# aschneuw/road-segmentation-unet

Hardware: AMD Instinct MI355X
Metric: 388x388 patches/sec fwd+bwd (1/2/4/8 GPU) + conv MFMA % of peak (higher is better)
Workload: dtype bf16; 1 GPU; U-Net fwd+bwd+momentum step, num_layers=5 root_size=64 patch_size=388 input=572; batch_per_gpu=4, global_batch=4, parallelism=dp1

## Files before the change

### road_segmentation_unet_amd/csrc/igemm.h

```cpp
#pragma once
#include "rsu_common.h"

struct IgSrc {
    const bf16_t* ptr;
    int H, W, C;
    int oy, ox;
};

struct IgFwdParams {
    IgSrc src[3];
    int nsrc;
    int nchunk[3];
    const bf16_t* wp;
    long wp_y_stride;
    int ntiles_w;
    int tile_off;
    const float* bias;
    bf16_t* out;
    const bf16_t* mask_src;
    bf16_t* pool_out;
    unsigned char* pool_code;
    const void* zero_page;
    int N, Hin, Win;
    int Ho, Wo;
    int Cout;
    int outC;
    int dil, stride, pad;
    int oH, oW, ostride;
    int relu, accumulate;
    int ncob;
    int lsw;
    int ksplit, cob_group;
    float* kslab;
    long kslab_stride;
    int dbg;
    unsigned* stamps;
    TileGeo g;
};

struct IgFwdCfgInfo { int TN, TM, threads; };
enum { IGF2_CFG_128x256 = 0, IGF2_CFG_64x512 = 1, IGF2_CFG_128x128 = 2, IGF2_CFG_64x256 = 3, IGF2_CFG_128x192 = 4, IGF2_CFG_64x384 = 5,
       IGF2_CFG_128x320 = 6, IGF2_CFG_64x640 = 7, IGF2_NCFG = 8 };
IgFwdCfgInfo igemm_fwd2_cfg_info(int cfg);
int igemm_fwd2_max_pieces(int cfg, int ntap);
size_t igemm_fwd2_lds_bytes(int cfg, int ntap, int npix_max);
hipError_t igemm_fwd2_launch(int cfg, int ntap, const IgFwdParams& p, int grid_x, int grid_y, hipStream_t st);
hipError_t igemm_pp_launch(int cfg, const IgFwdParams& p, int grid_x, hipStream_t st);
hipError_t igemm_pp_d2_launch(int cfg, const IgFwdParams& p, int grid_x, hipStream_t st);
bool igemm_pp_d2_supports(int cfg, const IgFwdParams& p);
bool igemm_pp_has(int cfg);
bool igemm_pp_has_ksplit(int cfg);
bool igemm_pp_supports(int cfg, const IgFwdParams& p);
int igemm_pp_pool_lsw_mask(int cfg);
size_t igemm_pp_slab_floats(int cfg, const IgFwdParams& p);
hipError_t igemm_pp_finish_launch(int cfg, const IgFwdParams& p, hipStream_t st);

struct IgCtParams {
    const bf16_t* a;
    int Ca;
    int nchunk;
    int N, H, W;
    unsigned magic_hw, magic_w;
    const bf16_t* wp;
    long wp_phase_stride;
    int ntiles_w;
    const float* bias;
    bf16_t* out;
    int outC;
    int Cn;
    const bf16_t* mask_src;
    int ncob, nnb;
};
bool igemm_ct_supports(int mode, int N, int H, int W, int Ca, int Cn);
hipError_t igemm_ct_launch(int mode, const IgCtParams& p, int grid_x, hipStream_t st);
hipError_t conv_first_fwd_launch(const void* in16, const void* wp, int ntiles_w, const float* bias, void* y, int N, int H, int W, int Cout, int dil,
                                 int relu, int ncu, hipStream_t st, const float* x = nullptr, const float* cw = nullptr, const float* cb = nullptr);

struct IgWgradParams {
    const bf16_t* F;
    int Hf, Wf, Cf;
    IgSrc S;
    float* slab;
    float* bslab;
    float* sbslab;
    long slab_stride;
    int CsOut, CfOut, cs_off;
    const void* zero_page;
    int N, dil, stride;
    int nsplit, ntiles_total;
    int lsw;
    int nbuf, nsw;
    int dbg;
    TileGeo g;
};
enum { IGW_CFG_64x64 = 0, IGW_CFG_64x16 = 1, IGW_CFG_128x64 = 2, IGW_NCFG = 3 };
size_t igemm_wgrad_lds_bytes(int cfg, int npix_max, int nbuf);
int igemm_wgrad_nsw(int cfg, int npix_max);
int igemm_wgrad_tmk(int cfg);
int igemm_wgrad_cfb(int cfg);
int igemm_wgrad_csb(int cfg);
int igemm_wgrad_kgroups(int cfg);
hipError_t igemm_wgrad_launch(int cfg, int ntap, const IgWgradParams& p, int grid_x, int grid_y, int grid_z,
                              hipStream_t st);
bool igemm_wgt_supports(int N, int H, int W, int Cin, int Cout);
int igemm_wgt_blocks(int Cin, int Cout);
int igemm_wgt_tiles(int N, int H, int W);
hipError_t igemm_wgt_launch(const void* x, const void* dy, float* slab, float* sbslab, long slab_stride, int N, int H, int W, int Cin, int Cout,
                            int nsplit, hipStream_t st);
bool igemm_wg1_supports(int N, int H, int W, int Cout, int dil);
int igemm_wg1_blocks(int Cout);
int igemm_wg1_tiles(int N, int Ho, int Wo);
hipError_t igemm_wg1_launch(const void* in16, const void* dz, float* slab, float* bslab, long slab_stride, int N, int H, int W, int Cout, int dil,
                            int nsplit, hipStream_t st);
enum { IGW_FAM_WGPP3 = 0, IGW_FAM_WGPP4 = 1, IGW_FAM_WGPP5 = 2, IGW_FAM_WGPP6 = 3, IGW_FAM_WGP64_4 = 4, IGW_FAM_WGP64_5 = 5,
       IGW_FAM_GENERIC = 8  };
#define IGW_GROUP_MAX 16
#define IGW_UNITS_MAX 2048
struct IgWgJob {
    IgWgradParams p;
    int gx, gy, gz;
    int family;
    int pad_;
};
struct IgWgGroupParams {
    int njobs, nwg;
    IgWgJob job[IGW_GROUP_MAX];
    int wg_first[257];
    unsigned unit[IGW_UNITS_MAX];
};
int igemm_wg_group_family(int cfg, int ntap, const IgWgradParams& p);
size_t igemm_wg_group_lds_bytes(int family, const IgWgradParams& p);
#define IGW_GROUP_LDS_BYTES (160 * 1024)
hipError_t igemm_wg_group_launch(const IgWgGroupParams* dev_table, int nwg_total, hipStream_t st);
bool igemm_wgpp_supports(int cfg, int ntap, const IgWgradParams& p);
bool igemm_wgp64_supports(int cfg, int ntap, const IgWgradParams& p);
hipError_t igemm_wgp64_launch(const IgWgradParams& p, int gx, int gy, int gz, hipStream_t st);
hipError_t igemm_wgpp_launch(const IgWgradParams& p, int grid_x, int grid_y, int grid_z, hipStream_t st);
```

### road_segmentation_unet_amd/csrc/igemm_ct.hip

```cpp
#include <type_traits>

#include "igemm.h"

#define RSU_SENT 0x80000000u

namespace {
__device__ __forceinline__ void bdma16c(__amdgpu_buffer_rsrc_t rsrc, unsigned voff, unsigned soff, void* lds_wave_base) {
    __builtin_amdgcn_raw_ptr_buffer_load_lds(rsrc, (__attribute__((address_space(3))) void*)lds_wave_base, 16, voff, soff, 0, 0);
}
}

template <int MODE>
__global__ void __launch_bounds__(512) __attribute__((amdgpu_waves_per_eu(2, 2))) igemm_ct_kernel(const IgCtParams p) {
    constexpr int NW = 8, CT = 4, PT = 4, TM = 256, TN = 128, WPX = 4;
    constexpr int APL = TM * 64, WPL = (TN / 16) * 1024;
    constexpr int SLOT = 2 * APL + 2 * WPL, NSLOT = 3;
    constexpr int NST = (CT / 2) * PT;
    constexpr int NPW = 6;
    extern __shared__ __attribute__((aligned(16))) char smem[];
    __attribute__((address_space(3))) char* lds = (__attribute__((address_space(3))) char*)smem;
    constexpr int bias_base = NSLOT * SLOT;

    const int lane = threadIdx.x & 63;
    const int wave = __builtin_amdgcn_readfirstlane(threadIdx.x >> 6);
    const int grp = wave >> 2, w4 = wave & 3;
    const int wco = wave / WPX, wpx = wave % WPX;
    const int g4 = lane >> 4, l15 = lane & 15, lq = lane >> 2;
    auto sgpr = [](auto v) { return __builtin_amdgcn_readfirstlane(v); };

    int vid = xcd_contiguous_id(blockIdx.x, gridDim.x);
    const int cob = vid % p.ncob;
    const int tile0 = vid / p.ncob, tstride = gridDim.x / p.ncob;
    const int M = p.N * p.H * p.W;
    const int ntile_m = (M + TM - 1) / TM;
    const int my_tiles = tile0 < ntile_m ? (ntile_m - tile0 + tstride - 1) / tstride : 0;
    if (my_tiles == 0) return;
    const int pha = MODE == 0 ? cob / p.nnb : 0, nb = MODE == 0 ? cob - pha * p.nnb : cob;
    const int ncols = MODE == 0 ? 2 * p.Cn : p.Cn;
    const int NS = MODE == 0 ? (p.nchunk + 1) / 2 : 4 * ((p.nchunk + 1) / 2);
    const int GS = my_tiles * NS;

    int boff[PT];
#pragma unroll
    for (int pt = 0; pt < PT; ++pt) {
        const int hp = (wpx * PT + pt) * 16 + l15;
        boff[pt] = (hp << 6) + ((g4 ^ ((hp >> 1) & 2)) << 4);
    }
    const int afrag = 2 * APL + (wco * CT * 64 + lane) * 16;
    auto mk = [&](const void* ptr) { return __builtin_amdgcn_make_buffer_rsrc((void*)ptr, 0, 0x7fffffff, 0x00020000); };

    const int wG = nb * 4 + w4;
    const bool wvalid = wG * 32 < ncols;
    unsigned w_base;
    if (MODE == 0) {
        const int b = (wG * 32) / p.Cn, lg = (wG * 32 - b * p.Cn) >> 5;
        w_base = sgpr((unsigned)(((long)(pha * 2 + b) * p.wp_phase_stride) * 2 + (long)lg * 2048));
    } else {
        w_base = sgpr((unsigned)(wG * 2048));
    }
    const unsigned w_blk = sgpr((unsigned)(p.ntiles_w * 1024));
    const unsigned w_lane = wvalid ? (unsigned)(lane * 16) : RSU_SENT;
    const int kg8 = ((lane & 3) ^ ((lq >> 1) & 2)) * 8;
    unsigned a_lane[MODE == 0 ? 1 : 4];
    if (MODE == 0) a_lane[0] = (unsigned)((lq * p.Ca + kg8) * 2);
    const int HW = p.H * p.W;
    auto pix_decode = [&](int m, int& n, int& y, int& x) {
        n = (int)__umulhi((unsigned)m, p.magic_hw);
        int r = m - n * HW;
        if (r >= HW) { ++n; r -= HW; }
        y = (int)__umulhi((unsigned)r, p.magic_w);
        x = r - y * p.W;
        if (x >= p.W) { ++y; x -= p.W; }
    };
    int pf_tile = 0;
    int pf_s = 0;
    int pf_slot = 0;
    auto pf_m0 = [&]() { return sgpr((tile0 + pf_tile * tstride) * TM); };
    auto pf_setup_tile = [&]() {
        if (MODE == 1) {
            const int m0 = pf_m0();
#pragma unroll
            for (int q = 0; q < 4; ++q) {
                const int m = m0 + (w4 * 4 + q) * 16 + lq;
                int n, y, x;
                pix_decode(m < M ? m : 0, n, y, x);
                a_lane[q] = m < M ? (unsigned)((((n * 2 * p.H + 2 * y) * 2 * p.W + 2 * x) * p.Ca + kg8) * 2) : RSU_SENT;
            }
        }
    };
    auto pf_issue = [&]() {
        const int st = MODE == 0 ? pf_s : (pf_s >> 2) ;
        const int tap = MODE == 0 ? 0 : (pf_s & 3);
        const int chunk = 2 * st + grp;
        const bool cvalid = chunk < p.nchunk;
        const int crem = p.Ca - chunk * 32;
        const __amdgpu_buffer_rsrc_t ra = mk(p.a), rw = mk(p.wp);
        const int dstA = pf_slot * SLOT + grp * APL, dstW = pf_slot * SLOT + 2 * APL + grp * WPL;
        const int m0 = pf_m0();
        if (MODE == 0) {
            const unsigned soff = sgpr((unsigned)(((long)(m0 + w4 * 64) * p.Ca + chunk * 32) * 2));
            const unsigned pstep = (unsigned)(16 * p.Ca * 2);
            const bool full = cvalid && crem >= 32 && m0 + TM <= M;
#pragma unroll
            for (int q = 0; q < 4; ++q) {
                unsigned vo = a_lane[0];
                if (!full) vo = (cvalid && kg8 < crem && m0 + (w4 * 4 + q) * 16 + lq < M) ? a_lane[0] : RSU_SENT;
                bdma16c(ra, vo, soff + q * pstep, (void*)(lds + dstA + (w4 * 4 + q) * 1024));
            }
        } else {
            const int ta = tap >> 1, tb = tap & 1;
            const unsigned soff = sgpr((unsigned)(((ta * 2 * p.W + tb) * p.Ca + chunk * 32) * 2));
            const bool full = cvalid && crem >= 32;
#pragma unroll
            for (int q = 0; q < 4; ++q) {
                unsigned vo = a_lane[q];
                if (!full) vo = (cvalid && kg8 < crem) ? a_lane[q] : RSU_SENT;
                bdma16c(ra, vo, soff, (void*)(lds + dstA + (w4 * 4 + q) * 1024));
            }
        }
        {
            const unsigned soff = sgpr(w_base + (unsigned)(MODE == 0 ? chunk : chunk * 4 + tap) * w_blk);
            const unsigned vo = cvalid ? w_lane : RSU_SENT;
            bdma16c(rw, vo, soff, (void*)(lds + dstW + (w4 * 2) * 1024));
            bdma16c(rw, vo == RSU_SENT ? RSU_SENT : vo + 1024, soff, (void*)(lds + dstW + (w4 * 2 + 1) * 1024));
        }
        pf_slot = pf_slot == NSLOT - 1 ? 0 : pf_slot + 1;
        if (++pf_s == NS) {
            pf_s = 0;
            if (pf_tile + 1 < my_tiles) ++pf_tile;
            pf_setup_tile();
        }
    };

    if (threadIdx.x < TN) {
        const int col = nb * TN + threadIdx.x;
        float bv = 0.f;
        if (MODE == 0 && p.bias && col < ncols) bv = p.bias[col >= p.Cn ? col - p.Cn : col];
        *(__attribute__((address_space(3))) float*)(lds + bias_base + threadIdx.x * 4) = bv;
    }
    asm volatile("s_waitcnt vmcnt(0)" ::: "memory");
#define CT_STORE(R, VOFF) \
    asm volatile("s_nop 4\n\tbuffer_store_dwordx4 %0, %1, %2, %3 offen\n\ts_nop 3" ::"v"(R), "v"(VOFF), "s"(orsrc), "s"(sbase) : "memory")
    unsigned ovoff[PT];
    const int colw = nb * TN + wco * (CT / 2) * 32;
    auto epi_setup_tile = [&](int m0) {
#pragma unroll
        for (int pt = 0; pt < PT; ++pt) {
            const int m = m0 + (wpx * PT + pt) * 16 + l15;
            if (MODE == 0) {
                int n, y, x;
                pix_decode(m < M ? m : 0, n, y, x);
                ovoff[pt] = m < M ? (unsigned)((((n * 2 * p.H + 2 * y + pha) * 2 * p.W + 2 * x) * p.outC + colw + 8 * g4) * 2) : RSU_SENT;
            } else {
                ovoff[pt] = m < M ? (unsigned)((((wpx * PT + pt) * 16 + l15) * p.outC + colw + 8 * g4) * 2) : RSU_SENT;
            }
        }
    };
    auto epilogue = [&](int m0, f32x4(&acc)[CT][PT]) {
        const __amdgpu_buffer_rsrc_t orsrc = mk(p.out);
        const __amdgpu_buffer_rsrc_t mrsrc = mk(p.mask_src ? (const void*)p.mask_src : (const void*)p.out);
        const unsigned sbase = MODE == 0 ? 0u : sgpr((unsigned)((long)m0 * p.outC * 2));
        unsigned ones_pk = 0x00010001u;
        asm volatile("" : "+v"(ones_pk));
        unsigned voffs[NST];
        u32x4 mk4[NST];
#pragma unroll
        for (int e = 0; e < NST; ++e) {
            const int pt = e / (CT / 2), pp = e % (CT / 2);
            const bool cok = colw + pp * 32 + 8 * g4 < ncols;
            voffs[e] = (cok && ovoff[pt] != RSU_SENT) ? ovoff[pt] + pp * 64 : RSU_SENT;
        }
        if (MODE == 1 && p.mask_src) {
#pragma unroll
            for (int e = 0; e < NST; ++e) mk4[e] = __builtin_amdgcn_raw_buffer_load_b128(mrsrc, voffs[e], sbase, 0);
        }
#pragma unroll
        for (int e = 0; e < NST; ++e) {
            const int pt = e / (CT / 2), pp = e % (CT / 2);
            u32x4 r;
#pragma unroll
            for (int i = 0; i < 2; ++i) {
                r[i] = pack_bf2(acc[2 * pp][pt][2 * i], acc[2 * pp][pt][2 * i + 1]);
                r[2 + i] = pack_bf2(acc[2 * pp + 1][pt][2 * i], acc[2 * pp + 1][pt][2 * i + 1]);
            }
            if (MODE == 1 && p.mask_src) {
#pragma unroll
                for (int i = 0; i < 4; ++i) r[i] &= pos_mask_pk_bf16(mk4[e][i], ones_pk);
            }
            CT_STORE(r, voffs[e]);
        }
    };
    auto bar = [&]() {
        asm volatile("" ::: "memory");
        __builtin_amdgcn_s_barrier();
        asm volatile("" ::: "memory");
    };

    pf_setup_tile();
    pf_issue();
    pf_issue();
    asm volatile("s_waitcnt vmcnt(0) lgkmcnt(0)" ::: "memory");
    bar();
    if (grp) bar();

    f32x4 acc[CT][PT];
    auto run_stream = [&](auto gconst) {
        constexpr int G = decltype(gconst)::value;
        int sit = 0;
        int ck = 0;
        bool after_epi = false;
        epi_setup_tile((tile0 + 0 * tstride) * TM);
        auto phase = [&](auto slotc) {
            constexpr int SL = decltype(slotc)::value;
            if (sit == 0) {
#pragma unroll
                for (int ct = 0; ct < CT; ++ct) {
                    const f32x4 bv = *(const __attribute__((address_space(3))) f32x4*)(lds + bias_base +
                                                                                         ((wco * (CT / 2) + (ct >> 1)) * 32 + 8 * g4 + (ct & 1) * 4) * 4);
#pragma unroll
                    for (int pt = 0; pt < PT; ++pt) {
                        acc[ct][pt] = bv;
                        asm volatile("" : "+v"(acc[ct][pt]));
                    }
                }
            }
            bf16x8 fa[2][CT], fb[2][PT];
#pragma unroll
            for (int ks = 0; ks < 2; ++ks) {
#pragma unroll
                for (int ct = 0; ct < CT; ++ct)
                    fa[ks][ct] = *(const __attribute__((address_space(3))) bf16x8*)(lds + afrag + (SL * SLOT + ks * WPL + ct * 1024));
#pragma unroll
                for (int pt = 0; pt < PT; ++pt)
                    fb[ks][pt] = *(const __attribute__((address_space(3))) bf16x8*)(lds + boff[pt] + (SL * SLOT + ks * APL));
            }
            pf_issue();
            if constexpr (G == 1) {
                if (after_epi) asm volatile("s_waitcnt vmcnt(%0)" ::"n"(NPW + NST) : "memory");
                else asm volatile("s_waitcnt vmcnt(%0)" ::"n"(NPW) : "memory");
            }
            asm volatile("s_waitcnt lgkmcnt(0)" ::: "memory");
            bar();
            __builtin_amdgcn_sched_barrier(0);
            __builtin_amdgcn_s_setprio(1);
#pragma unroll
            for (int ks = 0; ks < 2; ++ks)
#pragma unroll
                for (int pt = 0; pt < PT; ++pt)
#pragma unroll
                    for (int ct = 0; ct < CT; ++ct) mfma_bf16_inplace(acc[ct][pt], fa[ks][ct], fb[ks][pt]);
            __builtin_amdgcn_s_setprio(0);
            __builtin_amdgcn_sched_barrier(0);
            if constexpr (G == 0) {
                if (after_epi) asm volatile("s_waitcnt vmcnt(%0)" ::"n"(NPW + NST) : "memory");
                else asm volatile("s_waitcnt vmcnt(%0)" ::"n"(NPW) : "memory");
            }
            after_epi = false;
            if (sit == NS - 1) mfma_results_fence();
            bar();
            if (sit == NS - 1) {
                const int m0 = sgpr((tile0 + ck * tstride) * TM);
                epilogue(m0, acc);
                after_epi = true;
                sit = 0;
                ++ck;
                if (ck < my_tiles) epi_setup_tile((tile0 + ck * tstride) * TM);
            } else {
                ++sit;
            }
        };
        for (int gs = 0; gs < GS; gs += 3) {
            phase(std::integral_constant<int, 0>{});
            if (gs + 1 >= GS) break;
            phase(std::integral_constant<int, 1>{});
            if (gs + 2 >= GS) break;
            phase(std::integral_constant<int, 2>{});
        }
    };
    if (grp) run_stream(std::integral_constant<int, 1>{}); else run_stream(std::integral_constant<int, 0>{});
    if (!grp) bar();
    asm volatile("s_waitcnt vmcnt(0)" ::: "memory");
}

static size_t ct_lds_bytes() { return 3 * (2 * 256 * 64 + 2 * 8 * 1024) + 512; }

template <int MODE>
static hipError_t ct_launch_one(const IgCtParams& p, int gx, hipStream_t st) {
    auto kern = igemm_ct_kernel<MODE>;
    static bool set = false;
    if (!set) {
        hipError_t e = hipFuncSetAttribute((const void*)kern, hipFuncAttributeMaxDynamicSharedMemorySize, (int)ct_lds_bytes());
        if (e != hipSuccess) return e;
        set = true;
    }
    hipLaunchKernelGGL(kern, dim3(gx), dim3(512), ct_lds_bytes(), st, p);
    return hipGetLastError();
}
bool igemm_ct_supports(int mode, int N, int H, int W, int Ca, int Cn) {
    if (mode == 0 && (Cn % 32)) return false;
    return (long)N * H * W < (1L << 24) && Ca % 8 == 0 && Cn % 8 == 0 && H >= 1 && W >= 1;
}
hipError_t igemm_ct_launch(int mode, const IgCtParams& p, int gx, hipStream_t st) {
    return mode == 0 ? ct_launch_one<0>(p, gx, st) : ct_launch_one<1>(p, gx, st);
}
```

### road_segmentation_unet_amd/csrc/rsu_api.hip

```cpp
#include <array>
#include <atomic>
#include <cmath>
#include <cstdlib>
#include <cstring>
#include <algorithm>
#include <cstddef>
#include <map>
#include <mutex>
#include <vector>

#include "../../include/rsu.h"
#include "../../include/rsu_optim.h"
#include "../../include/rsu_loss.h"
#include "../../include/rsu_cldice.h"
#include "../../include/rsu_lovasz.h"
#include "../../include/rsu_components.h"
#include "../../include/rsu_distance.h"
#include "../../include/rsu_thin.h"
#include "affine_patches.h"
#include "color_jitter.h"
#include "border_map.h"
#include "elementwise.h"
#include "head.h"
#include "cldice.h"
// ... 690 lines not shown
            } ev;
            HIP_CHECK_RET(hipEventCreate(&ev.a));
            HIP_CHECK_RET(hipEventCreate(&ev.b));
            const hipEvent_t e0 = ev.a, e1 = ev.b;
            HIP_CHECK_RET(hipDeviceSynchronize());
            float best_ms = 1e30f, model_ms = 1e30f;
            int best_cfg = pl2.cfg | (pp << 8);
            const int model_code = best_cfg;
            for (int cfg = 0; cfg < IGF2_NCFG; ++cfg) {
                if (igemm_fwd2_cfg_info(cfg).TN != tn_model) continue;
                Fwd2Plan pc;
                if (!plan_fwd2(pc, ncu, N, Ho, Wo, Cout, ntap, kh, kw, dil, stride, gy, ktot, cfg, pool)) continue;
                IgFwdParams pt = p;
                apply_plan(pt, pc);
                for (int vpp = 0; vpp < 2; ++vpp) {
                    if (vpp == 1 && !(pp_ok && !accumulate && pp_supports(cfg, pt))) continue;
                    if (vpp == 0 && pool) continue;
                    if (!vpp && gen >= 4 && pp_ok && !accumulate && pp_supports(cfg, pt)) continue;
                    float ms_min = 1e30f;
                    for (int rep = 0; rep < 6; ++rep) {
                        HIP_CHECK_RET(hipEventRecord(e0, st));
                        HIP_CHECK_RET(launch_persistent(vpp, pc.cfg, ntap, pt, pc.grid_x, gy, st));
                        HIP_CHECK_RET(hipEventRecord(e1, st));
                        HIP_CHECK_RET(hipEventSynchronize(e1));
                        float ms = 0.f;
                        HIP_CHECK_RET(hipEventElapsedTime(&ms, e0, e1));
                        if (rep > 0 && ms < ms_min) ms_min = ms;
                    }
                    if (env_int("RSU_PLAN_DEBUG", 0)) fprintf(stderr, "[tune fwd2] cfg%d pp%d %.1f us\n", cfg, vpp, ms_min * 1e3f);
                    const int code = cfg | (vpp << 8);
                    if (code == model_code) model_ms = ms_min;
                    if (ms_min < best_ms) {
                        best_ms = ms_min;
                        best_cfg = code;
                    }
                }
            }
            if (best_ms > 0.97f * model_ms) best_cfg = model_code;
            if (env_int("RSU_PLAN_DEBUG", 0)) fprintf(stderr, "[tune fwd2] model cfg%d pp%d -> measured cfg%d pp%d\n", pl2.cfg, (int)pp, best_cfg & 255, best_cfg >> 8);
            std::lock_guard<std::mutex> lk(g_tune_mutex);
            g_tuned[tkey] = best_cfg;
            return RSU_OK;
        }
        HIP_CHECK_RET(launch_persistent(pp, pl2.cfg, ntap, p, pl2.grid_x, gy, st));
        return RSU_OK;
    }
}

extern "C" size_t rsu_conv_splitk_ws_floats(void) { return (size_t)256 * 128 * 256 + 1024; }
extern "C" int rsu_conv2d_fwd_k(const rsu_src_t* srcs, int nsrc, const void* packed_fwd, const float* bias, void* y, int N, int Hin,
                                int Win, int Cout, int dil, int relu, int ncu, float* kws, size_t kws_floats, rsu_stream_t stream) {
    if (!srcs || nsrc < 1 || nsrc > 3 || !packed_fwd || !y || Cout % 8 || (dil != 1 && dil != 2)) return RSU_EINVAL;
    const int Ho = Hin - 2 * dil, Wo = Win - 2 * dil;
    if (Ho < 1 || Wo < 2) return RSU_EINVAL;
    return run_fwd(srcs, nsrc, packed_fwd, 0, rup(Cout, 128) / 16, 0, bias, y, nullptr, N, Hin, Win, Ho, Wo, Cout, Cout, 9, 3, dil, 1, 0,
                   Ho, Wo, 1, 1, relu, 0, ncu, (hipStream_t)stream, nullptr, nullptr, kws, kws_floats);
}
extern "C" int rsu_conv2d_fwd(const rsu_src_t* srcs, int nsrc, const void* packed_fwd, const float* bias, void* y, int N, int Hin,
                              int Win, int Cout, int dil, int relu, int ncu, rsu_stream_t stream) {
    return rsu_conv2d_fwd_k(srcs, nsrc, packed_fwd, bias, y, N, Hin, Win, Cout, dil, relu, ncu, nullptr, 0, stream);
}

extern "C" int rsu_conv2d_fwd_pool_k(const rsu_src_t* srcs, int nsrc, const void* packed_fwd, const float* bias, void* y, void* pooled, void* code,
                                     int N, int Hin, int Win, int Cout, float keep, unsigned key, int ncu, float* kws, size_t kws_floats, rsu_stream_t stream);
extern "C" int rsu_conv2d_fwd_pool(const rsu_src_t* srcs, int nsrc, const void* packed_fwd, const float* bias, void* y, void* pooled, void* code,
                                   int N, int Hin, int Win, int Cout, float keep, unsigned key, int ncu, rsu_stream_t stream) {
    return rsu_conv2d_fwd_pool_k(srcs, nsrc, packed_fwd, bias, y, pooled, code, N, Hin, Win, Cout, keep, key, ncu, nullptr, 0, stream);
}
extern "C" int rsu_conv2d_fwd_pool_k(const rsu_src_t* srcs, int nsrc, const void* packed_fwd, const float* bias, void* y, void* pooled, void* code,
                                     int N, int Hin, int Win, int Cout, float keep, unsigned key, int ncu, float* kws, size_t kws_floats, rsu_stream_t stream) {
    if (!srcs || nsrc < 1 || nsrc > 3 || !packed_fwd || !y || !pooled || Cout % 8 || !keep_ok(keep)) return RSU_EINVAL;
    const int Ho = Hin - 2, Wo = Win - 2;
    if (Ho < 2 || Wo < 2) return RSU_EINVAL;
    if (code && ((Ho | Wo) & 1)) return RSU_EINVAL;
    const bool even = ((Ho | Wo) & 1) == 0;
    const int fuse = env_int("RSU_POOL_FUSED", 1);
    bool worth = fuse >= 2;
    if (fuse == 1) {
        Fwd2Plan a, b;
        const int n = launch_ncu(ncu), kt = 0;
        int ktot = 0;
        for (int i = 0; i < nsrc; ++i) ktot += rup(srcs[i].C, 32) * 9;
        (void)kt;
        Fwd2Plan sp;
        worth = n > 0 && !(kws && plan_split(sp, N, Ho, Wo, Cout, ktot, kws_floats)) &&
                plan_fwd2(a, n, N, Ho, Wo, Cout, 9, 3, 3, 1, 1, 1, ktot, -1, false) &&
                plan_fwd2(b, n, N, Ho, Wo, Cout, 9, 3, 3, 1, 1, 1, ktot, -1, true) && b.cost <= 1.08 * a.cost;
    }
    if (keep == 1.f && even && worth && env_int("RSU_FWD_GEN", 3) >= 3 && env_int("RSU_FWD2_CFG", -1) < 0) {
        const int rc = run_fwd(srcs, nsrc, packed_fwd, 0, rup(Cout, 128) / 16, 0, bias, y, nullptr, N, Hin, Win, Ho, Wo, Cout, Cout, 9, 3, 1, 1, 0, Ho, Wo,
                               1, 1, 1, 0, ncu, (hipStream_t)stream, pooled, code);
        if (rc != RSU_EINVAL) return rc;
    }
    const int rc = rsu_conv2d_fwd_k(srcs, nsrc, packed_fwd, bias, y, N, Hin, Win, Cout, 1, 1, ncu, kws, kws_floats, stream);
    if (rc != RSU_OK) return rc;
    return rsu_maxpool2x2_fwd_code(y, pooled, code, N, Ho, Wo, Cout, keep, key, stream);
}

extern "C" size_t rsu_packed_first_bytes(int Cout) {
    int seg[1] = {3};
    return rsu_packed_bytes(9, Cout, seg, 1);
}
extern "C" int rsu_pack_conv_first(const float* w, void* packed, int Cout, rsu_stream_t stream) {
    int seg[1] = {3};
    return do_pack(w, packed, 9, Cout, seg, 1, (long)3 * Cout, 1, Cout, 0, (hipStream_t)stream);
}
extern "C" int rsu_conv_first_fwd(const void* in16, const void* packed, const float* b, void* y, int N, int H, int W, int Cout, int dil,
                                  int ncu, rsu_stream_t stream) {
    if (!in16 || !packed || !y || Cout % 8 || H <= 2 * dil || W <= 2 * dil + 1 || (dil != 1 && dil != 2)) return RSU_EINVAL;
    rsu_src_t s;
    s.ptr = in16; s.H = H; s.W = W; s.C = 16; s.oy = 0; s.ox = 0;
    const int Ho = H - 2 * dil, Wo = W - 2 * dil;
    if (env_int("RSU_FIRST_GEN", 1) != 0) {
        const int n = launch_ncu(ncu);
        if (n < 0) return RSU_EINVAL;
        if ((long)N * Ho * Wo * Cout * 2 >= 0x7ffffff0L || (long)N * H * W * 32 >= 0x7ffffff0L) return RSU_E2BIG;
        HIP_CHECK_RET(conv_first_fwd_launch(in16, packed, rup(Cout, 128) / 16, b, y, N, H, W, Cout, dil, 1, n, (hipStream_t)stream));
        return RSU_OK;
    }
    return run_fwd(&s, 1, packed, 0, rup(Cout, 128) / 16, 0, b, y, nullptr, N, H, W, Ho, Wo, Cout, Cout, 9, 3, dil, 1, 0, Ho, Wo, 1, 1, 1, 0,
                   ncu, (hipStream_t)stream);
}

extern "C" int rsu_color_conv_first_fwd(const float* x, const float* w0, const float* b0, const void* packed, const float* b, void* y, int N, int H,
                                        int W, int Cout, int dil, int ncu, rsu_stream_t stream) {
    if (!x || !w0 || !b0 || !packed || !y || Cout % 8 || H <= 2 * dil || W <= 2 * dil + 1 || (dil != 1 && dil != 2)) return RSU_EINVAL;
    const int Ho = H - 2 * dil, Wo = W - 2 * dil;
    const int n = launch_ncu(ncu);
    if (n < 0) return RSU_EINVAL;
    if ((long)N * Ho * Wo * Cout * 2 >= 0x7ffffff0L || (long)N * H * W * 12 >= 0x7ffffff0L) return RSU_E2BIG;
    HIP_CHECK_RET(conv_first_fwd_launch(nullptr, packed, rup(Cout, 128) / 16, b, y, N, H, W, Cout, dil, 1, n, (hipStream_t)stream, x, w0, b0));
    return RSU_OK;
}

extern "C" int rsu_conv2d_bwd_data_k(const void* dz, const void* packed_bwd, void* dx, const void* relu_src, int accumulate, int N, int H,
                                     int W, int Cin_total, int ci_off, int ci_cnt, int Cout, int dil, int ncu, float* kws, size_t kws_floats, rsu_stream_t stream);
extern "C" int rsu_conv2d_bwd_data(const void* dz, const void* packed_bwd, void* dx, const void* relu_src, int accumulate, int N, int H,
                                   int W, int Cin_total, int ci_off, int ci_cnt, int Cout, int dil, int ncu, rsu_stream_t stream) {
    return rsu_conv2d_bwd_data_k(dz, packed_bwd, dx, relu_src, accumulate, N, H, W, Cin_total, ci_off, ci_cnt, Cout, dil, ncu, nullptr, 0, stream);
}
extern "C" int rsu_conv2d_bwd_data_k(const void* dz, const void* packed_bwd, void* dx, const void* relu_src, int accumulate, int N, int H,
                                     int W, int Cin_total, int ci_off, int ci_cnt, int Cout, int dil, int ncu, float* kws, size_t kws_floats, rsu_stream_t stream) {
    if (!dz || !packed_bwd || !dx || Cout % 8 || ci_cnt % 8 || ci_off % 32 || ci_off + ci_cnt > Cin_total || (dil != 1 && dil != 2))
        return RSU_EINVAL;
    const int Hd = H - 2 * dil, Wd = W - 2 * dil;
    if (Hd < 1 || Wd < 1 || W < 2) return RSU_EINVAL;
    rsu_src_t s;
    s.ptr = dz; s.H = Hd; s.W = Wd; s.C = Cout; s.oy = 0; s.ox = 0;
    return run_fwd(&s, 1, packed_bwd, 0, rup(Cin_total, 128) / 16, ci_off / 16, nullptr, dx, relu_src, N, Hd, Wd, H, W, ci_cnt, ci_cnt, 9,
                   3, dil, 1, 2 * dil, H, W, 1, 1, 0, accumulate, ncu, (hipStream_t)stream, nullptr, nullptr, kws, kws_floats);
}

static unsigned magic_floor32(int d) { return d <= 1 ? 0xffffffffu : (unsigned)(0x100000000ull / (unsigned)d); }
static int run_ct(int mode, const void* a, int Ca, int N, int H, int W, const void* wp, long phase_stride, int ntiles_w, const float* bias,
                  void* out, int outC, int Cn, const void* mask_src, int ncu_arg, hipStream_t st) {
    const int ncu = launch_ncu(ncu_arg);
    if (ncu < 0) return RSU_EINVAL;
    IgCtParams p;
    memset(&p, 0, sizeof(p));
    p.a = (const bf16_t*)a;
    p.Ca = Ca;
    p.nchunk = cdiv(Ca, 32);
    p.N = N; p.H = H; p.W = W;
    p.magic_hw = magic_floor32(H * W);
    p.magic_w = magic_floor32(W);
    p.wp = (const bf16_t*)wp;
    p.wp_phase_stride = phase_stride;
    p.ntiles_w = ntiles_w;
    p.bias = bias;
    p.out = (bf16_t*)out;
    p.outC = outC;
    p.Cn = Cn;
    p.mask_src = (const bf16_t*)mask_src;
    p.nnb = cdiv((mode == 0 ? 2 : 1) * Cn, 128);
    p.ncob = (mode == 0 ? 2 : 1) * p.nnb;
    const int ntile_m = cdiv(N * H * W, 256);
    int cols = ncu / p.ncob;
    if (cols < 1) cols = 1;
    if (cols > ntile_m) cols = ntile_m;
    HIP_CHECK_RET(igemm_ct_launch(mode, p, cols * p.ncob, st));
    return RSU_OK;
}

extern "C" int rsu_convT2x2_fwd(const void* x, const void* packed_fwd, const float* bias, void* y, int N, int H, int W, int Cin, int Cout,
                                int ncu, rsu_stream_t stream) {
    if (!x || !packed_fwd || !y || Cin % 8 || Cout % 8 || W < 2) return RSU_EINVAL;
    rsu_src_t s;
    s.ptr = x; s.H = H; s.W = W; s.C = Cin; s.oy = 0; s.ox = 0;
    int seg[1] = {Cin};
    const long per = (long)(rsu_packed_bytes(1, Cout, seg, 1) / 2);
    if (env_int("RSU_CT_GEN", 2) >= 2 && igemm_ct_supports(0, N, H, W, Cin, Cout) && (long)N * 4 * H * W * Cout * 2 < 0x7ffffff0L)
        return run_ct(0, x, Cin, N, H, W, packed_fwd, per, rup(Cout, 128) / 16, bias, y, Cout, Cout, nullptr, ncu, (hipStream_t)stream);
    return run_fwd(&s, 1, packed_fwd, per, rup(Cout, 128) / 16, 0, bias, y, nullptr, N, H, W, H, W, Cout, Cout, 1, 1, 1, 1, 0, 2 * H, 2 * W,
                   2, 4, 0, 0, ncu, (hipStream_t)stream);
}

extern "C" int rsu_convT2x2_bwd_data(const void* dy, const void* packed_bwd, void* dx, const void* relu_src, float out_scale, int N, int H,
                                     int W, int Cin, int Cout, int ncu, rsu_stream_t stream) {
    if (!dy || !packed_bwd || !dx || Cin % 8 || Cout % 8 || W < 2 || !(out_scale > 0.f)) return RSU_EINVAL;
    rsu_src_t s;
    s.ptr = dy; s.H = 2 * H; s.W = 2 * W; s.C = Cout; s.oy = 0; s.ox = 0;
    const bool ct = env_int("RSU_CT_GEN", 2) >= 2 && igemm_ct_supports(1, N, H, W, Cout, Cin) && (long)N * 4 * H * W * Cout * 2 < 0x7ffffff0L;
    const int rc = ct ? run_ct(1, dy, Cout, N, H, W, packed_bwd, 0, rup(Cin, 128) / 16, nullptr, dx, Cin, Cin, relu_src, ncu, (hipStream_t)stream)
                      : run_fwd(&s, 1, packed_bwd, 0, rup(Cin, 128) / 16, 0, nullptr, dx, relu_src, N, 2 * H, 2 * W, H, W, Cin, Cin, 4, 2, 1, 2, 0,
                                H, W, 1, 1, 0, 0, ncu, (hipStream_t)stream);
    if (rc != RSU_OK || out_scale == 1.f) return rc;
    HIP_CHECK_RET(ew_scale_bf16(dx, (long)N * H * W * Cin, out_scale, (hipStream_t)stream));
    return RSU_OK;
}

static int wgrad_pick_cfg(int cfg, int Cf) {
    if (cfg == IGW_CFG_64x64 && Cf >= 128 && env_int("RSU_WG_CFG", IGW_CFG_128x64) == IGW_CFG_128x64) return IGW_CFG_128x64;
    return cfg;
}
static int wgrad_max_split(int cfg, int Cf, int Cs, int ncu = 256) {
    int want = ncu / (cdiv(Cf, igemm_wgrad_cfb(cfg)) * cdiv(Cs, igemm_wgrad_csb(cfg)));
    return want < 1 ? 1 : want;
}
static size_t wgrad_max_slabs(int cfg, int Cf, int Cs) {
    const int a = wgrad_max_split(cfg, Cf, Cs), b = wgrad_max_split(wgrad_pick_cfg(cfg, Cf), Cf, Cs);
    return (size_t)(a > b ? a : b);
}
struct WgPlan { int cfg; TileGeo g; int gx, gy, nsplit, ntiles, lsw, nbuf; };
static bool plan_wgrad(WgPlan& pl, int ncu, int cfg, int N, int Hf, int Wf, int Cf, int Cs, int ntap, int kh, int kw, int dil, int stride) {
    pl.cfg = cfg;
    const int csb = igemm_wgrad_csb(cfg), cfbk = igemm_wgrad_cfb(cfg);
    const int tmk = igemm_wgrad_tmk(cfg);
    bool ok = false;
    for (int nbuf = 3; nbuf >= 2 && !ok; --nbuf) {
        const long fixed = (long)nbuf * tmk * 2 * cfbk;
        if (fixed >= 150 * 1024) continue;
        int cap = (int)((160 * 1024 - fixed) / (nbuf * csb * 2));
        const int ppw = 64 / (csb / 8) * 8;
        cap = cap / ppw * ppw;
        const int cap5 = 5 * ppw;
        if (nbuf == 3 && cap > cap5) cap = cap5;
        if (cap < ppw) continue;
        pl.nbuf = nbuf;
        ok = plan_geo_aligned(pl.g, pl.lsw, Hf, Wf, tmk, kh, kw, dil, stride, cap);
    }
    if (!ok) return false;
    pl.gx = cdiv(Cf, cfbk);
    pl.gy = cdiv(Cs, csb);
    pl.ntiles = N * pl.g.nstrips * pl.g.tiles_per_strip;
    const int want = wgrad_max_split(cfg, Cf, Cs, ncu);
    pl.nsplit = want < pl.ntiles ? want : pl.ntiles;
    (void)ntap;
    return true;
}

struct WgPrep {
    int cfg, ntap, gx, gy, ntiles, extra;
    long main_elems;
    IgWgradParams p;
    float *out, *db, *dbs;
    int cs_cnt;
};
static int prep_wgrad(WgPrep& w, int cfg, const void* F, int Hf, int Wf, int Cf, const rsu_src_t* S, float* out, int CsOut, int CfOut,
                      int cs_off, int N, int ntap, int kw, int dil, int stride, int ncu, float* db, float* dbs) {
    if ((long)N * Hf * Wf * Cf * 2 >= 0x7ffffff0L || (long)N * S->H * S->W * S->C * 2 >= 0x7ffffff0L) return RSU_E2BIG;
    WgPlan pl;
    const int wide = wgrad_pick_cfg(cfg, Cf);
    if (wide != cfg && plan_wgrad(pl, ncu, wide, N, Hf, Wf, Cf, S->C, ntap, ntap / kw, kw, dil, stride)) cfg = wide;
    else if (!plan_wgrad(pl, ncu, cfg, N, Hf, Wf, Cf, S->C, ntap, ntap / kw, kw, dil, stride)) return RSU_EINVAL;
    if (db && dbs) return RSU_EINVAL;
    if (dbs && (CsOut % 4 || cs_off != 0 || S->C != CsOut)) return RSU_EINVAL;
    IgWgradParams& p = w.p;
    memset(&p, 0, sizeof(p));
    p.F = (const bf16_t*)F;
    p.Hf = Hf; p.Wf = Wf; p.Cf = Cf;
    p.S.ptr = (const bf16_t*)S->ptr;
    p.S.H = S->H; p.S.W = S->W; p.S.C = S->C; p.S.oy = S->oy; p.S.ox = S->ox;
    p.CsOut = CsOut; p.CfOut = CfOut; p.cs_off = cs_off;
    p.zero_page = zero_page();
    if (!p.zero_page) return RSU_EHIP;
    p.N = N; p.dil = dil; p.stride = stride;
    p.nsplit = pl.nsplit;
    p.ntiles_total = pl.ntiles;
    p.lsw = pl.lsw;
    p.nbuf = pl.nbuf;
    p.nsw = igemm_wgrad_nsw(cfg, pl.g.npix_max);
#ifdef RSU_DEV_KERNELS
    p.dbg = env_int("RSU_WG_DBG", 0);
#endif
    p.g = pl.g;
    w.cfg = cfg; w.ntap = ntap; w.gx = pl.gx; w.gy = pl.gy; w.ntiles = pl.ntiles;
    w.main_elems = (long)ntap * CsOut * CfOut;
    w.extra = db ? CfOut : (dbs ? rup(CsOut, 4) : 0);
    w.out = out; w.db = db; w.dbs = dbs; w.cs_cnt = S->C;
    return RSU_OK;
}
static void finish_wgrad(WgPrep& w, int nsplit, float* ws) {
    IgWgradParams& p = w.p;
    p.nsplit = nsplit;
    p.slab = nsplit == 1 ? w.out : ws;
    p.slab_stride = w.main_elems + w.extra;
    p.bslab = w.db ? (nsplit == 1 ? w.db : ws + w.main_elems) : nullptr;
    p.sbslab = w.dbs ? (nsplit == 1 ? w.dbs : ws + w.main_elems) : nullptr;
}
static int run_wgrad(int cfg, const void* F, int Hf, int Wf, int Cf, const rsu_src_t* S, float* out, float* ws, int CsOut, int CfOut,
                     int cs_off, int N, int ntap, int kw, int dil, int stride, int ncu_arg, hipStream_t st, float* db = nullptr, float* dbs = nullptr) {
    const int ncu = launch_ncu(ncu_arg);
    if (ncu < 0) return RSU_EINVAL;
    WgPrep w;
    const int rc = prep_wgrad(w, cfg, F, Hf, Wf, Cf, S, out, CsOut, CfOut, cs_off, N, ntap, kw, dil, stride, ncu, db, dbs);
    if (rc != RSU_OK) return rc;
    const int nslab = w.p.nsplit;
    finish_wgrad(w, nslab, ws);
    const IgWgradParams& p = w.p;
    if (env_int("RSU_WG_GEN", 2) >= 2 && igemm_wgpp_supports(w.cfg, ntap, p))
        HIP_CHECK_RET(igemm_wgpp_launch(p, w.gx, w.gy, nslab, st));
    else if (env_int("RSU_WG_GEN", 2) >= 2 && env_int("RSU_WG64", 1) && igemm_wgp64_supports(w.cfg, ntap, p))
        HIP_CHECK_RET(igemm_wgp64_launch(p, w.gx, w.gy, nslab, st));
    else
        HIP_CHECK_RET(igemm_wgrad_launch(w.cfg, ntap, p, w.gx, w.gy, nslab, st));
    if (nslab > 1) {
        HIP_CHECK_RET(ew_reduce_slabs(ws, out, db ? db : dbs, w.extra / 4, nslab, p.slab_stride, ntap, CsOut, cs_off, S->C, CfOut, st));
    }
    return RSU_OK;
}

extern "C" size_t rsu_conv2d_bwd_weight_ws_floats(int Cin_total, int src_C, int Cout) {
    return wgrad_max_slabs(IGW_CFG_64x64, Cout, src_C) * (9 * (size_t)Cin_total * Cout + Cout);
}
extern "C" int rsu_conv2d_bwd_weight(const rsu_src_t* src, const void* dz, float* dw, float* db, float* ws, int N, int Ho, int Wo,
                                     int Cin_total, int ci_off, int Cout, int dil, int ncu, rsu_stream_t stream) {
    if (!src || !src->ptr || !dz || !dw || !ws || src->C % 8 || Cout % 8 || ci_off + src->C > Cin_total || (dil != 1 && dil != 2))
        return RSU_EINVAL;
    if (src->oy < 0 || src->ox < 0 || src->oy + Ho + 2 * dil > src->H || src->ox + Wo + 2 * dil > src->W || Wo < 2) return RSU_EINVAL;
    return run_wgrad(IGW_CFG_64x64, dz, Ho, Wo, Cout, src, dw, ws, Cin_total, Cout, ci_off, N, 9, 3, dil, 1, ncu, (hipStream_t)stream, db);
}

extern "C" size_t rsu_convT2x2_bwd_weight_ws_floats(int Cin, int Cout) {
// ... 726 lines not shown
```

Baseline: 968.7 patches/s.

## Add 128-pixel tile variant and cost-model tile choice for transposed-conv kernel

Templates the 2x2 transposed-conv igemm kernel on pixel tile size (128 or 256) and picks the tile per layer with a cycle cost model based on wave rounds, stage count and per-tile overhead. It also adds a lane-transposed store path that uses ds_bpermute so each lane writes contiguous channels, enabled by default except for forward mode with the 128 tile. Mask loads are issued early through inline asm so they overlap the packing. The goal is better CU utilisation on small deep layers where 256-pixel tiles leave the grid underfilled, at the cost of more template instances and cost-model constants hand-tuned to this chip.

```diff
diff --git a/road_segmentation_unet_amd/csrc/igemm.h b/road_segmentation_unet_amd/csrc/igemm.h
--- a/road_segmentation_unet_amd/csrc/igemm.h
+++ b/road_segmentation_unet_amd/csrc/igemm.h
@@ -71,8 +71,16 @@
     const bf16_t* mask_src;
     int ncob, nnb;
 };
+#define CT_LAUNCH 21200
+#define CT_INTERVAL_256 690
+#define CT_TILE_FWD_256 5400
+#define CT_TILE_BWD_256 8600
+#define CT_INTERVAL_128 540
+#define CT_TILE_FWD_128 2700
+#define CT_TILE_BWD_128 4400
+#define CT_MERGED_STORES(mode, tm) (!((mode) == 0 && (tm) == 128))
 bool igemm_ct_supports(int mode, int N, int H, int W, int Ca, int Cn);
-hipError_t igemm_ct_launch(int mode, const IgCtParams& p, int grid_x, hipStream_t st);
+hipError_t igemm_ct_launch(int mode, int tm, int trs, const IgCtParams& p, int grid_x, hipStream_t st);
 hipError_t conv_first_fwd_launch(const void* in16, const void* wp, int ntiles_w, const float* bias, void* y, int N, int H, int W, int Cout, int dil,
                                  int relu, int ncu, hipStream_t st, const float* x = nullptr, const float* cw = nullptr, const float* cb = nullptr);
 
diff --git a/road_segmentation_unet_amd/csrc/igemm_ct.hip b/road_segmentation_unet_amd/csrc/igemm_ct.hip
--- a/road_segmentation_unet_amd/csrc/igemm_ct.hip
+++ b/road_segmentation_unet_amd/csrc/igemm_ct.hip
@@ -10,13 +10,15 @@
 }
 }
 
-template <int MODE>
+template <int MODE, int TM, bool TRS>
 __global__ void __launch_bounds__(512) __attribute__((amdgpu_waves_per_eu(2, 2))) igemm_ct_kernel(const IgCtParams p) {
-    constexpr int NW = 8, CT = 4, PT = 4, TM = 256, TN = 128, WPX = 4;
+    static_assert(TM == 128 || TM == 256, "pixel tile");
+    constexpr int NW = 8, CT = 4, WPX = 4, PT = TM / (16 * WPX), TN = 128;
+    constexpr int NAP = TM / 64;
     constexpr int APL = TM * 64, WPL = (TN / 16) * 1024;
     constexpr int SLOT = 2 * APL + 2 * WPL, NSLOT = 3;
     constexpr int NST = (CT / 2) * PT;
-    constexpr int NPW = 6;
+    constexpr int NPW = NAP + 2;
     extern __shared__ __attribute__((aligned(16))) char smem[];
     __attribute__((address_space(3))) char* lds = (__attribute__((address_space(3))) char*)smem;
     constexpr int bias_base = NSLOT * SLOT;
@@ -26,6 +28,7 @@
     const int grp = wave >> 2, w4 = wave & 3;
     const int wco = wave / WPX, wpx = wave % WPX;
     const int g4 = lane >> 4, l15 = lane & 15, lq = lane >> 2;
+    const int el15 = TRS ? lq : l15, eg4 = TRS ? (lane & 3) : g4;
     auto sgpr = [](auto v) { return __builtin_amdgcn_readfirstlane(v); };
 
     int vid = xcd_contiguous_id(blockIdx.x, gridDim.x);
@@ -61,7 +64,7 @@
     const unsigned w_blk = sgpr((unsigned)(p.ntiles_w * 1024));
     const unsigned w_lane = wvalid ? (unsigned)(lane * 16) : RSU_SENT;
     const int kg8 = ((lane & 3) ^ ((lq >> 1) & 2)) * 8;
-    unsigned a_lane[MODE == 0 ? 1 : 4];
+    unsigned a_lane[MODE == 0 ? 1 : NAP];
     if (MODE == 0) a_lane[0] = (unsigned)((lq * p.Ca + kg8) * 2);
     const int HW = p.H * p.W;
     auto pix_decode = [&](int m, int& n, int& y, int& x) {
@@ -80,8 +83,8 @@
         if (MODE == 1) {
             const int m0 = pf_m0();
 #pragma unroll
-            for (int q = 0; q < 4; ++q) {
-                const int m = m0 + (w4 * 4 + q) * 16 + lq;
+            for (int q = 0; q < NAP; ++q) {
+                const int m = m0 + (w4 * NAP + q) * 16 + lq;
                 int n, y, x;
                 pix_decode(m < M ? m : 0, n, y, x);
                 a_lane[q] = m < M ? (unsigned)((((n * 2 * p.H + 2 * y) * 2 * p.W + 2 * x) * p.Ca + kg8) * 2) : RSU_SENT;
@@ -98,24 +101,24 @@
         const int dstA = pf_slot * SLOT + grp * APL, dstW = pf_slot * SLOT + 2 * APL + grp * WPL;
         const int m0 = pf_m0();
         if (MODE == 0) {
-            const unsigned soff = sgpr((unsigned)(((long)(m0 + w4 * 64) * p.Ca + chunk * 32) * 2));
+            const unsigned soff = sgpr((unsigned)(((long)(m0 + w4 * NAP * 16) * p.Ca + chunk * 32) * 2));
             const unsigned pstep = (unsigned)(16 * p.Ca * 2);
             const bool full = cvalid && crem >= 32 && m0 + TM <= M;
 #pragma unroll
-            for (int q = 0; q < 4; ++q) {
+            for (int q = 0; q < NAP; ++q) {
                 unsigned vo = a_lane[0];
-                if (!full) vo = (cvalid && kg8 < crem && m0 + (w4 * 4 + q) * 16 + lq < M) ? a_lane[0] : RSU_SENT;
-                bdma16c(ra, vo, soff + q * pstep, (void*)(lds + dstA + (w4 * 4 + q) * 1024));
+                if (!full) vo = (cvalid && kg8 < crem && m0 + (w4 * NAP + q) * 16 + lq < M) ? a_lane[0] : RSU_SENT;
+                bdma16c(ra, vo, soff + q * pstep, (void*)(lds + dstA + (w4 * NAP + q) * 1024));
             }
         } else {
             const int ta = tap >> 1, tb = tap & 1;
             const unsigned soff = sgpr((unsigned)(((ta * 2 * p.W + tb) * p.Ca + chunk * 32) * 2));
             const bool full = cvalid && crem >= 32;
 #pragma unroll
-            for (int q = 0; q < 4; ++q) {
+            for (int q = 0; q < NAP; ++q) {
                 unsigned vo = a_lane[q];
                 if (!full) vo = (cvalid && kg8 < crem) ? a_lane[q] : RSU_SENT;
-                bdma16c(ra, vo, soff, (void*)(lds + dstA + (w4 * 4 + q) * 1024));
+                bdma16c(ra, vo, soff, (void*)(lds + dstA + (w4 * NAP + q) * 1024));
             }
         }
         {
@@ -146,13 +149,13 @@
     auto epi_setup_tile = [&](int m0) {
 #pragma unroll
         for (int pt = 0; pt < PT; ++pt) {
-            const int m = m0 + (wpx * PT + pt) * 16 + l15;
+            const int m = m0 + (wpx * PT + pt) * 16 + el15;
             if (MODE == 0) {
                 int n, y, x;
                 pix_decode(m < M ? m : 0, n, y, x);
-                ovoff[pt] = m < M ? (unsigned)((((n * 2 * p.H + 2 * y + pha) * 2 * p.W + 2 * x) * p.outC + colw + 8 * g4) * 2) : RSU_SENT;
+                ovoff[pt] = m < M ? (unsigned)((((n * 2 * p.H + 2 * y + pha) * 2 * p.W + 2 * x) * p.outC + colw + 8 * eg4) * 2) : RSU_SENT;
             } else {
-                ovoff[pt] = m < M ? (unsigned)((((wpx * PT + pt) * 16 + l15) * p.outC + colw + 8 * g4) * 2) : RSU_SENT;
+                ovoff[pt] = m < M ? (unsigned)((((wpx * PT + pt) * 16 + el15) * p.outC + colw + 8 * eg4) * 2) : RSU_SENT;
             }
         }
     };
@@ -164,26 +167,42 @@
         asm volatile("" : "+v"(ones_pk));
         unsigned voffs[NST];
         u32x4 mk4[NST];
+        const int tr_src = (((lane & 3) << 4) | (lane >> 2)) << 2;
 #pragma unroll
         for (int e = 0; e < NST; ++e) {
             const int pt = e / (CT / 2), pp = e % (CT / 2);
-            const bool cok = colw + pp * 32 + 8 * g4 < ncols;
+            const bool cok = colw + pp * 32 + 8 * eg4 < ncols;
             voffs[e] = (cok && ovoff[pt] != RSU_SENT) ? ovoff[pt] + pp * 64 : RSU_SENT;
         }
-        if (MODE == 1 && p.mask_src) {
-#pragma unroll
-            for (int e = 0; e < NST; ++e) mk4[e] = __builtin_amdgcn_raw_buffer_load_b128(mrsrc, voffs[e], sbase, 0);
-        }
+        const bool masked = MODE == 1 && p.mask_src;
+        if (masked) {
+#pragma unroll
+            for (int e = 0; e < NST; ++e)
+                asm volatile("buffer_load_dwordx4 %0, %1, %2, %3 offen" : "=&v"(mk4[e]) : "v"(voffs[e]), "s"(mrsrc), "s"(sbase) : "memory");
+        }
+        u32x4 rr[NST];
 #pragma unroll
         for (int e = 0; e < NST; ++e) {
             const int pt = e / (CT / 2), pp = e % (CT / 2);
-            u32x4 r;
 #pragma unroll
             for (int i = 0; i < 2; ++i) {
-                r[i] = pack_bf2(acc[2 * pp][pt][2 * i], acc[2 * pp][pt][2 * i + 1]);
-                r[2 + i] = pack_bf2(acc[2 * pp + 1][pt][2 * i], acc[2 * pp + 1][pt][2 * i + 1]);
-            }
-            if (MODE == 1 && p.mask_src) {
+                rr[e][i] = pack_bf2(acc[2 * pp][pt][2 * i], acc[2 * pp][pt][2 * i + 1]);
+                rr[e][2 + i] = pack_bf2(acc[2 * pp + 1][pt][2 * i], acc[2 * pp + 1][pt][2 * i + 1]);
+            }
+            if (TRS) {
+#pragma unroll
+                for (int i = 0; i < 4; ++i) rr[e][i] = (unsigned)__builtin_amdgcn_ds_bpermute(tr_src, (int)rr[e][i]);
+            }
+        }
+        if (masked) {
+            asm volatile("s_waitcnt vmcnt(0)" ::: "memory");
+#pragma unroll
+            for (int e = 0; e < NST; ++e) asm volatile("" : "+v"(mk4[e]));
+        }
+#pragma unroll
+        for (int e = 0; e < NST; ++e) {
+            u32x4 r = rr[e];
+            if (masked) {
 #pragma unroll
                 for (int i = 0; i < 4; ++i) r[i] &= pos_mask_pk_bf16(mk4[e][i], ones_pk);
             }
@@ -282,24 +301,28 @@
     asm volatile("s_waitcnt vmcnt(0)" ::: "memory");
 }
 
-static size_t ct_lds_bytes() { return 3 * (2 * 256 * 64 + 2 * 8 * 1024) + 512; }
-
-template <int MODE>
+static size_t ct_lds_bytes(int tm) { return 3 * (2 * (size_t)tm * 64 + 2 * 8 * 1024) + 512; }
+
+template <int MODE, int TM, bool TRS>
 static hipError_t ct_launch_one(const IgCtParams& p, int gx, hipStream_t st) {
-    auto kern = igemm_ct_kernel<MODE>;
+    auto kern = igemm_ct_kernel<MODE, TM, TRS>;
     static bool set = false;
     if (!set) {
-        hipError_t e = hipFuncSetAttribute((const void*)kern, hipFuncAttributeMaxDynamicSharedMemorySize, (int)ct_lds_bytes());
+        hipError_t e = hipFuncSetAttribute((const void*)kern, hipFuncAttributeMaxDynamicSharedMemorySize, (int)ct_lds_bytes(TM));
         if (e != hipSuccess) return e;
         set = true;
     }
-    hipLaunchKernelGGL(kern, dim3(gx), dim3(512), ct_lds_bytes(), st, p);
+    hipLaunchKernelGGL(kern, dim3(gx), dim3(512), ct_lds_bytes(TM), st, p);
     return hipGetLastError();
 }
 bool igemm_ct_supports(int mode, int N, int H, int W, int Ca, int Cn) {
     if (mode == 0 && (Cn % 32)) return false;
     return (long)N * H * W < (1L << 24) && Ca % 8 == 0 && Cn % 8 == 0 && H >= 1 && W >= 1;
 }
-hipError_t igemm_ct_launch(int mode, const IgCtParams& p, int gx, hipStream_t st) {
-    return mode == 0 ? ct_launch_one<0>(p, gx, st) : ct_launch_one<1>(p, gx, st);
-}
+hipError_t igemm_ct_launch(int mode, int tm, int trs, const IgCtParams& p, int gx, hipStream_t st) {
+    if (tm != 128 && tm != 256) return hipErrorInvalidValue;
+#define CT_PICK(M, T) (trs ? ct_launch_one<M, T, true>(p, gx, st) : ct_launch_one<M, T, false>(p, gx, st))
+    if (tm == 128) return mode == 0 ? CT_PICK(0, 128) : CT_PICK(1, 128);
+    return mode == 0 ? CT_PICK(0, 256) : CT_PICK(1, 256);
+#undef CT_PICK
+}
diff --git a/road_segmentation_unet_amd/csrc/rsu_api.hip b/road_segmentation_unet_amd/csrc/rsu_api.hip
--- a/road_segmentation_unet_amd/csrc/rsu_api.hip
+++ b/road_segmentation_unet_amd/csrc/rsu_api.hip
@@ -866,6 +866,26 @@
 }
 
 static unsigned magic_floor32(int d) { return d <= 1 ? 0xffffffffu : (unsigned)(0x100000000ull / (unsigned)d); }
+static const int CT_INTERVAL[2] = {CT_INTERVAL_128, CT_INTERVAL_256};
+static const int CT_TILE[2][2] = {{CT_TILE_FWD_128, CT_TILE_FWD_256}, {CT_TILE_BWD_128, CT_TILE_BWD_256}};
+static long ct_model_cycles(int mode, long M, int Ca, int Cn, int ncu, int tm) {
+    const int ncob = cdiv((mode == 0 ? 2 : 1) * Cn, 128) * (mode == 0 ? 2 : 1);
+    const long ntile = (M + tm - 1) / tm;
+    long cols = ncu / ncob;
+    if (cols < 1) cols = 1;
+    if (cols > ntile) cols = ntile;
+    const long rounds = (ntile + cols - 1) / cols;
+    const long stages = (mode == 0 ? 1 : 4) * cdiv(cdiv(Ca, 32), 2);
+    return CT_LAUNCH + rounds * (stages * 2 * CT_INTERVAL[tm == 256] + CT_TILE[mode][tm == 256]);
+}
+static int ct_plan_tm(int mode, long M, int Ca, int Cn, int ncu) {
+    return ct_model_cycles(mode, M, Ca, Cn, ncu, 128) < ct_model_cycles(mode, M, Ca, Cn, ncu, 256) ? 128 : 256;
+}
+extern "C" int rsu_dev_convT_plan_tm(int mode, int N, int H, int W, int Ca, int Cn, int ncu) {
+    const int n = launch_ncu(ncu);
+    if (n < 0 || (mode != 0 && mode != 1) || N < 1 || H < 1 || W < 1 || Ca < 1 || Cn < 1) return 0;
+    return ct_plan_tm(mode, (long)N * H * W, Ca, Cn, n);
+}
 static int run_ct(int mode, const void* a, int Ca, int N, int H, int W, const void* wp, long phase_stride, int ntiles_w, const float* bias,
                   void* out, int outC, int Cn, const void* mask_src, int ncu_arg, hipStream_t st) {
     const int ncu = launch_ncu(ncu_arg);
@@ -888,11 +908,17 @@
     p.mask_src = (const bf16_t*)mask_src;
     p.nnb = cdiv((mode == 0 ? 2 : 1) * Cn, 128);
     p.ncob = (mode == 0 ? 2 : 1) * p.nnb;
-    const int ntile_m = cdiv(N * H * W, 256);
+    int tm = env_int("RSU_CT_TM", 0);
+    if (tm != 128 && tm != 256) tm = ct_plan_tm(mode, (long)N * H * W, Ca, Cn, ncu);
+    const int ntile_m = cdiv(N * H * W, tm);
     int cols = ncu / p.ncob;
     if (cols < 1) cols = 1;
     if (cols > ntile_m) cols = ntile_m;
-    HIP_CHECK_RET(igemm_ct_launch(mode, p, cols * p.ncob, st));
+    if (env_int("RSU_PLAN_DEBUG", 0))
+        fprintf(stderr, "[plan ct] mode%d M %d Ca %d Cn %d ncu %d tm%d grid %d\n", mode, N * H * W, Ca, Cn, ncu, tm, cols * p.ncob);
+    int trs = env_int("RSU_CT_STORE", -1);
+    if (trs != 0 && trs != 1) trs = CT_MERGED_STORES(mode, tm);
+    HIP_CHECK_RET(igemm_ct_launch(mode, tm, trs, p, cols * p.ncob, st));
     return RSU_OK;
 }
 
```

After: 973.0 patches/s (median of 5 runs). No clear change (+0.4%).
